# facebookresearch/param

Hardware: AMD Instinct MI355X
Metric: EmbeddingBag lookups/s + achieved HBM GB/s; all-to-all bus-BW at 1/2/4/8 GPU (higher is better)
Workload: dtype f32

## Files before the change

param_amd/csrc/bwd_sorted_alt.inc:

```
#include <rocprim/device/device_radix_sort.hpp>

namespace pm {
namespace {

template <typename K, bool WEIGHTED>
__global__ void __launch_bounds__(kBlock) build_keys_kernel(const KParams p, K* keys, uint32_t* vals,
                                                            uint32_t* bag_of, int rbits, int tshift, int kbits,
                                                            int64_t phase_bags, int64_t slice_begin, int64_t slice_end) {
    extern __shared__ __attribute__((aligned(16))) char smem[];
    int t, tile;
    block_to_tile(p, t, tile);
    if (t >= p.T) return;
    const int64_t bag0 = static_cast<int64_t>(tile) * p.bags_per_block;
    const int64_t left = p.B - bag0;
    const int nb = left < p.bags_per_block ? static_cast<int>(left) : p.bags_per_block;
    const int64_t g0 = static_cast<int64_t>(t) * p.B + bag0;
    int64_t* s_off = reinterpret_cast<int64_t*>(smem);
    for (int i = threadIdx.x; i <= nb; i += kBlock) s_off[i] = bag_start_or_end(p, g0 + i);
    __syncthreads();
    const int64_t base = s_off[0];
    const int64_t end = s_off[nb];
    const K pad = static_cast<K>(1) << kbits;
    for (int64_t j = base + threadIdx.x; j < end; j += kBlock) {
        int lo = 0, hi = nb;
        while (hi - lo > 1) {
            const int mid = (lo + hi) >> 1;
            if (s_off[mid] <= j) lo = mid; else hi = mid;
        }
        const int64_t bag = bag0 + lo;
        const K row = static_cast<K>(load_index(p.indices, j, p.idx64));
        const bool in_slice = bag >= slice_begin && bag < slice_end;
        const K phase = phase_bags > 0 ? static_cast<K>(bag / phase_bags) : static_cast<K>(0);
        keys[j] = in_slice ? ((static_cast<K>(t) << tshift) | (phase << rbits) | row) : pad;
        if (WEIGHTED) {
            vals[j] = static_cast<uint32_t>(j);
            bag_of[j] = static_cast<uint32_t>(bag);
        } else {
            vals[j] = static_cast<uint32_t>(bag);
        }
    }
}

template <typename K>
hipError_t rocprim_temp_bytes(int64_t n, int kbits_sort, size_t& bytes) {
    bytes = 0;
    K* kn = nullptr;
    uint32_t* vn = nullptr;
    return rocprim::radix_sort_pairs(nullptr, bytes, kn, kn, vn, vn, static_cast<size_t>(n), 0u,
                                     static_cast<unsigned>(kbits_sort), hipStream_t(0));
}

std::atomic<int> g_sort_impl{-1}, g_sort_order{-1}, g_max_phases{-1};
void set_alt_tuning(int sort_impl, int order, int max_phases_) {
    g_sort_impl.store(sort_impl);
    g_sort_order.store(order);
    g_max_phases.store(max_phases_);
}
int sort_impl_knob() { return knob(g_sort_impl, [] { return env_is("PARAM_AMD_SORT", "rocprim") ? 1 : env_is("PARAM_AMD_SORT", "legacy") ? 2 : 0; }); }
bool fused_keys_allowed() { return !env_is("PARAM_AMD_SORT_FUSED_KEYS", "0"); }
bool table_major_order() { return knob(g_sort_order, [] { return env_is("PARAM_AMD_SORT_ORDER", "row") ? 0 : 1; }) == 1; }
int max_phases() { return knob(g_max_phases, [] { return env_is("PARAM_AMD_BWD_PHASES", "2") ? 2 : 1; }); }

hipError_t alt_temp_bytes(int64_t n, int, int key_bytes, int kbits_sort, size_t& tb) {
    hipError_t rc = key_bytes == 4 ? rocprim_temp_bytes<uint32_t>(n, kbits_sort > 32 ? 32 : kbits_sort, tb)
                                   : rocprim_temp_bytes<uint64_t>(n, kbits_sort, tb);
    if (rc != hipSuccess) return rc;
    const size_t own = rs_scratch_bytes(static_cast<size_t>(n));
    if (own > tb) tb = own;
    return hipSuccess;
}

void legacy_plan(const KParams& p, int64_t fixed_pooling, int phases, SortPlan& g) {
    const bool fixed = fixed_pooling > 0 && !g.sliced && p.T >= 1 && p.B > 0 &&
                       fixed_pooling * p.B * static_cast<int64_t>(p.T) == p.N;
    g.H = 1;
    if (phases == 2 && max_phases() >= 2 && fixed && table_major_order() && p.B % 2 == 0 && ((p.B / 2) * fixed_pooling) % kSortTile == 0) g.H = 2;
    g.hbits = g.H == 2 ? 1 : 0;
    g.tshift = g.rbits + g.hbits;
    g.kbits = g.tshift + bits_for(p.T);
    g.key_bytes = (g.kbits + 1 <= 32) ? 4 : 8;
    g.phase_bags = g.H == 2 ? p.B / 2 : 0;
    g.seg_len = fixed ? (p.B / g.H) * fixed_pooling : 0;
    g.seg_tiles = (fixed && table_major_order() && g.seg_len % kSortTile == 0) ? static_cast<int32_t>(g.seg_len / kSortTile) : 0;
    g.segmented = fixed && table_major_order() && !g.rocprim && g.seg_len > 0 && g.seg_len % 4096 == 0 && g.seg_len / 4096 <= 4096;
    g.xcd = want_xcd() && g.seg_tiles > 0 && p.T > 1;
    if (g.sliced) g.sort_end_bit = g.kbits + 1;
    else if (g.segmented) g.sort_end_bit = g.rbits;
    else g.sort_end_bit = table_major_order() ? g.kbits : g.rbits;
    g.in_b = g.rocprim || (rs_num_passes(0, g.sort_end_bit) % 2 == 1);
    g.fused_keys = g.segmented && g.H == 1 && !g.weighted && !g.sliced && g.sort_end_bit > 0 && fused_keys_allowed();
}

template <typename K>
hipError_t legacy_sort(const KParams& p, const SortPlan& g, SortWs& ws, hipStream_t stream) {
    K* ka = reinterpret_cast<K*>(ws.keys_a);
    K* kb = reinterpret_cast<K*>(ws.keys_b);
    KParams q = p;
    q.bag_begin = 0;
    q.bag_count = p.B;
    q.tiles_per_table = static_cast<int32_t>((p.B + p.bags_per_block - 1) / p.bags_per_block);
    q.xcd_affine = 0;
    const int grid = q.T * q.tiles_per_table;
    const size_t lds = static_cast<size_t>(q.bags_per_block + 2) * sizeof(int64_t);
    hipError_t zrc = hipMemsetAsync(ws.fix_ctl, 0, 4 * sizeof(uint32_t), stream);
    if (zrc != hipSuccess) return zrc;
    const int64_t s0 = p.bag_begin, s1 = p.bag_begin + p.bag_count;
    if (g.fused_keys) {
        const RsSource src{p.indices, p.idx64, g.tshift, static_cast<uint32_t>(g.seg_len / p.B)};
        return rs_sort_pairs<K>(ka, kb, ws.vals_a, ws.vals_b, static_cast<size_t>(p.N), nullptr, 0, g.sort_end_bit, ws.temp, stream,
                                static_cast<size_t>(g.seg_len), &src);
    }
    if (g.weighted)
        hipLaunchKernelGGL((build_keys_kernel<K, true>), dim3(grid), dim3(kBlock), lds, stream, q, ka, ws.vals_a,
                           ws.bag_of, g.rbits, g.tshift, g.kbits, g.phase_bags, s0, s1);
    else
        hipLaunchKernelGGL((build_keys_kernel<K, false>), dim3(grid), dim3(kBlock), lds, stream, q, ka, ws.vals_a,
                           ws.bag_of, g.rbits, g.tshift, g.kbits, g.phase_bags, s0, s1);
    hipError_t rc = hipGetLastError();
    if (rc != hipSuccess) return rc;
    size_t tb = ws.temp_bytes;
    if (g.rocprim)
        return rocprim::radix_sort_pairs(ws.temp, tb, ka, kb, ws.vals_a, ws.vals_b, static_cast<size_t>(p.N), 0u,
                                         static_cast<unsigned>(g.sort_end_bit), stream);
    return rs_sort_pairs<K>(ka, kb, ws.vals_a, ws.vals_b, static_cast<size_t>(p.N), nullptr, 0, g.sort_end_bit, ws.temp, stream,
                            g.segmented ? static_cast<size_t>(g.seg_len) : 0);
}

std::string legacy_plan_describe(const SortPlan& g) {
    const int passes = g.rocprim ? -1 : rs_num_passes(0, g.sort_end_bit);
    char buf[640];
// ... 12 lines not shown
```

param_amd/csrc/bwd_sorted_apply.h:

```cpp
#pragma once

#include <type_traits>

#include "common.h"
#include "fwd_elem.h"

namespace pm {

constexpr int kSortTile = 1024;

constexpr int kExactRun = 256;
constexpr int kFixGrid = 2048;
constexpr int kMaxTablesLds = 1024;

struct ChunkRec {
    uint32_t lead_len;
    uint32_t trail_len;
};

constexpr uint32_t kJoinedBit = 0x80000000u;

struct SortedParams {
    ChunkRec* recs;
    uint32_t* fix_list;
    uint32_t* fix_ctl;
    float* partials;
    int32_t T;
    const void* keys;
    const uint32_t* vals;
    const uint32_t* bag_of;
    void* const* dst;
    const int32_t* dims;
    const int64_t* out_offsets;
    const float* grad;
    const float* psw;
    int64_t out_stride;
    int32_t gblk_shift;
    int64_t gblk_extra;
    int64_t n;
    int32_t rbits;
    int32_t kbits;
    int32_t max_dim;
    int32_t nt_rows;
    float alpha;
    float* const* mom;
    float lr;
    float eps;
    float wd;
    int32_t wd_mode;
    int32_t sr;
    uint64_t sr_seed;
    int32_t exact_run;
    int32_t tshift;
    int32_t seg_tiles;
    int32_t H;
    int32_t phase;
    int32_t tile;
    int32_t xcd;
    const uint32_t* d_n;
    int32_t unique_wgs_per_cu;
    int32_t join_tiles;
    float* const* state;
};


hipError_t bwd_sorted_launch_f32(const SortedParams& sp, int key_bytes, int max_dim, hipStream_t stream);
hipError_t bwd_sorted_launch_bf16(const SortedParams& sp, int key_bytes, int max_dim, hipStream_t stream);
hipError_t bwd_sorted_launch_f16(const SortedParams& sp, int key_bytes, int max_dim, hipStream_t stream);
struct UniqueArgs {
    const HybTable* hyb_tab;
    const uint32_t* bloom;
    void* emit_keys;
    uint32_t* emit_vals;
    int key_bytes;
    uint32_t* tile_cnt;
    size_t tile_cnt_stride;
    int bloom_wbits;
};
hipError_t bwd_unique_launch_f32(const SortedParams& sp, const KParams& kp, const UniqueArgs& ua, int max_dim, hipStream_t stream);
hipError_t bwd_unique_launch_bf16(const SortedParams& sp, const KParams& kp, const UniqueArgs& ua, int max_dim, hipStream_t stream);
hipError_t bwd_unique_launch_f16(const SortedParams& sp, const KParams& kp, const UniqueArgs& ua, int max_dim, hipStream_t stream);

struct RestArgs {
    const HybTable* hyb_tab;
    int T_h;
    const uint32_t* stage;
    const uint32_t* rest_n;
    const uint32_t* rbits;
    int rbits_stride;
    int parts;
};
int rest_parts(int T_h, int tiles_per_table);
hipError_t bwd_rest_launch_f32(const SortedParams& sp, const KParams& kp, const RestArgs& ra, int max_dim, hipStream_t stream);
hipError_t bwd_rest_launch_bf16(const SortedParams& sp, const KParams& kp, const RestArgs& ra, int max_dim, hipStream_t stream);
hipError_t bwd_rest_launch_f16(const SortedParams& sp, const KParams& kp, const RestArgs& ra, int max_dim, hipStream_t stream);

}
```

param_amd/csrc/embbag_bwd_sorted.hip:

```cpp
#include <atomic>
#include <climits>
#include <cstdint>
#include <cstdio>
#include <cstdlib>
#include <mutex>
#include <string>
#include <unordered_map>
#include <vector>

#include "bwd_sorted_apply.h"

namespace pm {
namespace {

constexpr int kDefaultSortMode = 0;

struct SortWs {
    char* keys_a;
    char* keys_b;
    uint32_t* vals_a;
    uint32_t* vals_b;
    uint32_t* bag_of;
    ChunkRec* recs;
    uint32_t* fix_list;
// ... 20 lines not shown
inline size_t align256(size_t x) { return (x + 255) / 256 * 256; }

inline int bits_for(int64_t n_values) {
    int b = 0;
    while ((static_cast<int64_t>(1) << b) < n_values) ++b;
    return b;
}

std::atomic<int> g_bwd_xcd{-1};
int env_is(const char* name, const char* value) {
    const char* e = getenv(name);
    return (e && std::string(e) == value) ? 1 : 0;
}
template <typename F>
int knob(std::atomic<int>& k, F env_default) {
    int v = k.load();
    if (v < 0) {
        v = env_default();
        k.store(v);
    }
    return v;
}
std::atomic<int> g_sort_mode{-1};
int sort_mode_knob() {
    int v = g_sort_mode.load();
    if (v < 0) {
        const char* e = getenv("PARAM_AMD_SORT_MODE");
        v = (e && e[0] >= '0' && e[0] <= '3') ? e[0] - '0' : kDefaultSortMode;
        g_sort_mode.store(v);
    }
    return v;
}
std::atomic<int> g_hyb_enable{-1};
std::atomic<uint32_t> g_spin_cap{0};
int env_int(const char* name, int dflt) {
    const char* e = getenv(name);
    return (e && e[0] >= '0' && e[0] <= '9') ? atoi(e) : dflt;
}
int hyb_enable_knob() { return knob(g_hyb_enable, [] { return env_int("PARAM_AMD_BWD_HYBRID", 1); }); }
std::atomic<int> g_hyb_rest{-1};
std::atomic<int> g_hyb_min_tiles{-1};
int hyb_rest_knob() { return knob(g_hyb_rest, [] { return env_int("PARAM_AMD_HYB_REST", 1) != 0 ? 1 : 0; }); }
bool want_xcd() { return knob(g_bwd_xcd, [] { return env_is("PARAM_AMD_BWD_XCD", "0") ? 0 : 1; }) == 1; }

struct SortPlan {
    int key_bytes, rbits, hbits, tshift, kbits;
    bool sliced, weighted, rocprim, segmented, in_b, xcd, fused_keys;
    int H;
    int64_t n, seg_len, phase_bags;
    int sort_end_bit;
    int32_t seg_tiles;
    int32_t T;
    bool v2;
    int mode;
    int hyb;
    bool applied;
    bool relabelled;
    bool sequence;
    const void* indices;
    const void* offsets;
    int64_t B, bag_begin, bag_count;
    uint64_t stamp;
};

}
}

#ifdef PM_ALTERNATES
#include "bwd_sorted_alt.inc"
#else
namespace pm {
namespace {
int sort_impl_knob() { return 0; }
void set_alt_tuning(int, int, int) {}
hipError_t alt_temp_bytes(int64_t, int T, int, int, size_t& tb) {
    tb = 0;
    return T > kSegSortMaxTables ? hipErrorInvalidValue : hipSuccess;
}
void legacy_plan(const KParams&, int64_t, int, SortPlan&) {}
template <typename K>
hipError_t legacy_sort(const KParams&, const SortPlan&, SortWs&, hipStream_t) { return hipErrorInvalidValue; }
std::string legacy_plan_describe(const SortPlan&) { return "sort=none"; }
}
}
#endif

namespace pm {
namespace {

template <typename F>
hipError_t with_key_type(int key_bytes, F&& f) {
    return key_bytes == 4 ? f(uint32_t{}) : f(uint64_t{});
}

SortWs ws_layout(const KParams& p, int64_t max_rows, int max_dim, bool weighted, void* base) {
    const int64_t n = p.N;
    const int kbits_sort = bits_for(max_rows) + 1 + bits_for(p.T) + 1;
    const int key_bytes = kbits_sort <= 32 ? 4 : 8;
    SortWs ws{};
    size_t tb = 0;
    if ((ws.rc = alt_temp_bytes(n, p.T, key_bytes, kbits_sort, tb)) != hipSuccess) return ws;
    if (p.T <= kSegSortMaxTables) {
        const size_t seg = seg_sort_scratch_bytes(static_cast<size_t>(n), p.T, !weighted);
        if (seg > tb) tb = seg;
    }
    char* b = reinterpret_cast<char*>(base);
    size_t off = 0;
    auto take = [&](size_t bytes) { char* q = b ? b + off : nullptr; off += align256(bytes); return q; };
    ws.keys_a = take(static_cast<size_t>(n) * key_bytes);
    ws.keys_b = take(static_cast<size_t>(n) * key_bytes);
    ws.vals_a = reinterpret_cast<uint32_t*>(take(static_cast<size_t>(n) * 4));
    ws.vals_b = reinterpret_cast<uint32_t*>(take(static_cast<size_t>(n) * 4));
    ws.bag_of = reinterpret_cast<uint32_t*>(take(weighted ? static_cast<size_t>(n) * 4 : 0));
    const size_t nch = static_cast<size_t>(max_chunks(n, max_dim));
    ws.recs = reinterpret_cast<ChunkRec*>(take(nch * sizeof(ChunkRec)));
    ws.fix_list = reinterpret_cast<uint32_t*>(take(nch * sizeof(uint32_t)));
    ws.fix_ctl = reinterpret_cast<uint32_t*>(take(4 * sizeof(uint32_t)));
    ws.partials = reinterpret_cast<float*>(take(nch * 2 * static_cast<size_t>(max_dim) * sizeof(float)));
    ws.temp = take(tb);
    ws.temp_bytes = tb;
    ws.total = off;
    return ws;
}

SortPlan make_plan(const KParams& p, int64_t max_rows, int64_t fixed_pooling, int phases, bool sequence = false) {
    SortPlan g;
    g.sequence = sequence;
    g.T = p.T;
    g.n = p.N;
    g.rbits = bits_for(max_rows);
    g.sliced = !(p.bag_begin == 0 && p.bag_count == p.B);
    g.weighted = p.psw != nullptr;
    g.rocprim = sort_impl_knob() == 1;
    g.indices = p.indices;
    g.offsets = p.offsets;
    g.B = p.B;
    g.bag_begin = p.bag_begin;
    g.bag_count = p.bag_count;
    g.stamp = 0;
    g.v2 = sort_impl_knob() == 0 && p.T <= kSegSortMaxTables;
    g.mode = sort_mode_knob();
    g.hyb = 0;
    g.applied = false;
    g.relabelled = false;
    g.H = 1;
    g.hbits = 0;
    g.tshift = g.rbits;
    g.kbits = g.tshift + bits_for(p.T);
    g.key_bytes = (g.kbits + 1 <= 32) ? 4 : 8;
    g.phase_bags = 0;
    g.seg_len = 0;
    g.seg_tiles = 0;
    g.segmented = g.v2;
    g.xcd = g.v2 && want_xcd();
    g.sort_end_bit = g.v2 ? g.rbits : g.kbits;
    g.in_b = g.v2 && seg_sort_result_in_b(g.mode, g.rbits);
    g.fused_keys = g.v2 && !g.weighted;
    if (!g.v2) legacy_plan(p, fixed_pooling, phases, g);
    return g;
}

std::mutex g_plan_mutex;
std::unordered_map<const void*, SortPlan> g_plans;
uint64_t g_plan_stamp = 0;

SegSortRequest seg_request(const KParams& p, const SortPlan& g, SortWs& ws) {
    SegSortRequest rq;
    rq.indices = p.indices;
    rq.offsets = p.offsets;
    rq.rows = p.rows;
    rq.idx64 = p.idx64;
    rq.T = p.T;
    rq.B = p.B;
    rq.N = p.N;
    rq.bag_begin = p.bag_begin;
    rq.bag_count = p.bag_count;
    rq.tshift = g.tshift;
    rq.rbits_max = g.rbits;
    rq.weighted = g.weighted;
    rq.sequence = g.sequence;
    rq.zero4 = ws.fix_ctl;
    rq.hyb.allow = g.hyb;
    rq.hyb.slices = hyb_slices(p.N, p.T);
    rq.queue_a = ws.vals_a;
    rq.queue_b = ws.vals_b;
    rq.spin_cap = g_spin_cap.load();
    return rq;
}

template <typename K>
hipError_t sort_impl(const KParams& p, const SortPlan& g, SortWs& ws, hipStream_t stream) {
    if (!g.v2) return legacy_sort<K>(p, g, ws, stream);
    const SegSortRequest rq = seg_request(p, g, ws);
    const hipError_t rc = seg_sort_part_a<K>(rq, ws.temp, stream);
    if (rc != hipSuccess || g.hyb) return rc;
    return seg_sort_part_b<K>(rq, g.mode, reinterpret_cast<K*>(ws.keys_a), reinterpret_cast<K*>(ws.keys_b), ws.vals_a, ws.vals_b, ws.bag_of,
                              ws.temp, stream);
}

template <typename F>
PlanStatus find_plan(const void* workspace, const KParams& p, int64_t max_rows, bool match, SortPlan& out, F&& follow_up) {
    std::lock_guard<std::mutex> lock(g_plan_mutex);
    auto it = g_plans.find(workspace);
    if (it == g_plans.end()) return PlanStatus::none;
    SortPlan& g = it->second;
// ... 108 lines not shown
}

PlanStatus sorted_pairs_info(const KParams& p, int64_t max_rows, int max_dim, const void* workspace, SortedPairsInfo& out) {
    SortPlan g;
    if (find_plan(workspace, p, max_rows, false, g, [](SortPlan&) { return PlanStatus::ok; }) != PlanStatus::ok) return PlanStatus::none;
    out.deferred = g.hyb && !g.applied;
    if (out.deferred) return PlanStatus::ok;
    const SortWs ws = ws_layout(p, max_rows, max_dim, g.weighted, const_cast<void*>(workspace));
    if (ws.rc != hipSuccess) return PlanStatus::none;
    out.keys = g.in_b ? ws.keys_b : ws.keys_a;
    out.vals = g.in_b ? ws.vals_b : ws.vals_a;
    out.d_count = g.v2 ? seg_sort_view(ws.temp, static_cast<size_t>(p.N), p.T).n_total : nullptr;
    out.key_bytes = g.key_bytes;
    out.tshift = g.tshift;
    return PlanStatus::ok;
}

hipError_t bwd_sorted_apply(const KParams& p, int64_t max_rows, int dst_dtype, int max_dim, const void* workspace, hipStream_t stream,
                            ApplyUpdate update) {
    SortPlan g;
    if (find_plan(workspace, p, max_rows, false, g, [](SortPlan& r) { r.applied = true; return PlanStatus::ok; }) != PlanStatus::ok)
        return hipErrorInvalidValue;
    SortWs ws = ws_layout(p, max_rows, max_dim, g.weighted, const_cast<void*>(workspace));
    if (ws.rc != hipSuccess) return ws.rc;
    if (p.T > kMaxTablesLds) return hipErrorInvalidValue;
    const SegScratchView sv = seg_sort_view(ws.temp, static_cast<size_t>(p.N), p.T);
    const pm_rowwise_adagrad* opt = update.opt;
    SortedParams sp;
    sp.recs = ws.recs;
    sp.fix_list = ws.fix_list;
    sp.fix_ctl = ws.fix_ctl;
    sp.partials = ws.partials;
    sp.T = p.T;
    sp.keys = g.in_b ? ws.keys_b : ws.keys_a;
    sp.vals = g.in_b ? ws.vals_b : ws.vals_a;
    sp.bag_of = ws.bag_of;
    sp.dst = const_cast<void* const*>(p.tables);
    sp.dims = p.dims;
    sp.out_offsets = g.sequence ? nullptr : p.out_offsets;
    sp.grad = p.io;
    sp.psw = p.psw;
    sp.out_stride = p.out_stride;
    sp.gblk_shift = p.gblk_shift;
    sp.gblk_extra = p.gblk_extra;
    sp.n = p.N;
    sp.rbits = g.rbits;
    sp.kbits = g.kbits;
    sp.tshift = g.tshift;
    sp.max_dim = max_dim;
    sp.nt_rows = p.nt_loads;
    sp.alpha = p.alpha;
    sp.mom = update.elementwise ? nullptr : update.state;
    sp.state = update.elementwise ? update.state : nullptr;
    sp.lr = opt ? opt->lr : 0.0f;
    sp.eps = opt ? opt->eps : 0.0f;
    sp.wd = opt ? opt->weight_decay : 0.0f;
    sp.wd_mode = opt ? opt->weight_decay_mode : PM_WD_NONE;
    sp.sr = (opt && opt->stochastic_rounding && dst_dtype != PM_F32) ? 1 : 0;
    sp.sr_seed = opt ? opt->seed : 0;
    sp.exact_run = kExactRun;
    sp.seg_tiles = (!g.v2 && (g.xcd || g.H > 1)) ? g.seg_tiles : 0;
    sp.H = g.H;
    sp.phase = 0;
    sp.xcd = g.xcd ? (g.v2 ? 2 : 1) : 0;
    sp.d_n = g.v2 ? sv.n_total : nullptr;
    sp.tile = g.v2 ? apply_tile(p.N) : kSortTile;
    sp.unique_wgs_per_cu = 0;
    if (sp.n == 0) return hipSuccess;
    const ApplyLaunchers& launch = kApplyLaunchers[dst_dtype == PM_F32 ? 0 : dst_dtype == PM_BF16 ? 1 : 2];
    if (g.sequence && (g.hyb || sp.psw || sp.gblk_extra != 0)) return hipErrorInvalidValue;
    if (!g.hyb) return launch.sorted(sp, g.key_bytes, max_dim, stream);
    UniqueArgs ua;
    ua.hyb_tab = sv.hyb_tab;
    ua.bloom = sv.bloom;
    ua.emit_keys = ws.keys_b;
    ua.emit_vals = ws.vals_b;
    ua.key_bytes = g.key_bytes;
    ua.tile_cnt = sv.tile_cnt;
    ua.tile_cnt_stride = sv.tile_cnt_stride;
    ua.bloom_wbits = bloom_wbits(hyb_slices(p.N, p.T));
    KParams q = p;
    q.bags_per_block = kUniqueBags;
    q.tiles_per_table = static_cast<int32_t>((q.bag_count + kUniqueBags - 1) / kUniqueBags);
    q.idx_cap = 4096;
    if (q.tiles_per_table < 1 || q.tiles_per_table > kCompactMaxTiles) return hipErrorInvalidValue;
    hipError_t rc = launch.unique(sp, q, ua, max_dim, stream);
    if (rc != hipSuccess) return rc;
    const int rest_mode = hyb_rest_knob();
    const HybTiles tiles{q.bags_per_block, q.tiles_per_table};
    rc = with_key_type(g.key_bytes, [&](auto k) {
        using K = decltype(k);
        return seg_sort_stage_leftovers<K>(seg_request(p, g, ws), reinterpret_cast<const K*>(ws.keys_b), ws.vals_b,
                                           reinterpret_cast<K*>(ws.keys_a), ws.vals_a, tiles, rest_mode != 0 ? 1 : 0, ws.temp, stream);
    });
    if (rc != hipSuccess) return rc;
    if (rest_mode != 0) {
        RestArgs ra;
        ra.hyb_tab = ua.hyb_tab;
        ra.T_h = p.T < kHybMaxTables ? p.T : kHybMaxTables;
        ra.stage = sv.rest_stage;
        ra.rest_n = sv.rest_n;
        ra.rbits = &sv.desc->rbits;
        ra.rbits_stride = static_cast<int>(sizeof(SegDesc) / sizeof(uint32_t));
        ra.parts = rest_parts(ra.T_h, q.tiles_per_table);
        if ((rc = launch.rest(sp, q, ra, max_dim, stream)) != hipSuccess) return rc;
    }
// ... 44 lines not shown
```

param_amd/csrc/embbag_bwd_sorted_kernels.inc:

```

template <typename DST, int G>
__device__ __forceinline__ void adagrad_finish(char* wptr, float (&wrow)[DST::kVec], const float (&acc)[DST::kVec],
                                               bool any_col, float* mom_row, float mom_prev, int D, const SortedParams& p,
                                               int lig, int nt_rows, uint64_t rowkey, int c) {
    float ss = 0.0f;
    if (p.wd_mode == PM_WD_L2) {
#pragma unroll
        for (int k = 0; k < DST::kVec; ++k) {
            const float reg = any_col ? p.wd * wrow[k] : 0.0f;
            const float gx = acc[k] + reg;
            ss = ss + gx * gx;
        }
    } else {
#pragma unroll
        for (int k = 0; k < DST::kVec; ++k) ss = ss + acc[k] * acc[k];
    }
#pragma unroll
    for (int off = G / 2; off >= 1; off >>= 1) ss = ss + __shfl_xor(ss, off, G);
    const float m = mom_prev + ss / static_cast<float>(D);
    if (lig == 0) hidden_store4(mom_row, m);
    const float mult = p.lr / (sqrtf(m) + p.eps);
    if (any_col) {
        if (p.wd_mode != PM_WD_NONE) {
            const float shrink = p.wd_mode == PM_WD_L2 ? mult * p.wd : p.lr * p.wd;
// ... 47 lines not shown
__device__ __forceinline__ void state_load_raw(const void* p, u32x4 (&raw)[VEC / 4], int nt_rows) {
#pragma unroll
    for (int k = 0; k < VEC / 4; ++k) raw[k] = raw16_load(reinterpret_cast<const char*>(p) + 16 * k, nt_rows);
}
template <int VEC>
__device__ __forceinline__ void state_widen(const u32x4 (&raw)[VEC / 4], float (&st)[VEC]) {
#pragma unroll
    for (int k = 0; k < VEC / 4; ++k) {
        st[4 * k] = __uint_as_float(raw[k].x); st[4 * k + 1] = __uint_as_float(raw[k].y);
        st[4 * k + 2] = __uint_as_float(raw[k].z); st[4 * k + 3] = __uint_as_float(raw[k].w);
    }
}

template <typename DST, int G, int OPT>
__device__ __forceinline__ void finish_row(char* wptr, float (&wrow)[DST::kVec], float (&acc)[DST::kVec], const float (&srow)[OPT == 2 ? DST::kVec : 1],
                                           bool cols, float* state, float m_prev, int D, const SortedParams& p, int lig, int nt_rows,
                                           uint64_t rowkey, int c) {
    if constexpr (OPT == 2) {
        if (cols) adagrad_elem_finish<DST>(wptr, wrow, acc, srow, state, p, nt_rows, rowkey, c);
    } else
    if (OPT == 1) adagrad_finish<DST, G>(wptr, wrow, acc, cols, state, m_prev, D, p, lig, nt_rows, rowkey, c);
    else if (cols) DST::store(wptr, acc, nt_rows);
}
template <int VEC, typename P>
__device__ __forceinline__ void load_grad(P g, float (&gv)[VEC]) {
#pragma unroll
    for (int k = 0; k < VEC; k += 4) {
        const f32x4 x = g[k / 4];
        gv[k] = x.x; gv[k + 1] = x.y; gv[k + 2] = x.z; gv[k + 3] = x.w;
    }
}
template <int VEC>
__device__ __forceinline__ void add_scaled(float (&acc)[VEC], float sc, const float (&gv)[VEC]) {
#pragma unroll
    for (int k = 0; k < VEC; ++k) {
        const float prod = sc * gv[k];
        acc[k] = acc[k] + prod;
    }
}
template <typename DST, int OPT>
__device__ __forceinline__ void open_row(const u32x4 raw, const u32x4 (&sraw)[OPT == 2 ? DST::kVec / 4 : 1], float (&acc)[DST::kVec],
                                         float (&wrow)[DST::kVec], float (&srow)[OPT == 2 ? DST::kVec : 1]) {
    float wv[DST::kVec];
    DST::widen(raw, wv);
#pragma unroll
    for (int k = 0; k < DST::kVec; ++k) {
        if (OPT != 0) wrow[k] = wv[k];
        else acc[k] = wv[k];
    }
    if constexpr (OPT == 2) state_widen<DST::kVec>(sraw, srow);
}
template <int OPT, int VEC>
__device__ __forceinline__ int column_pass_end(int lig, int width) { return OPT != 0 ? lig * VEC + 1 : width; }

template <int G>
__device__ __forceinline__ int group_first(bool pred) {
    const uint64_t m = __ballot(pred);
    if (G == 64) return m ? __builtin_ctzll(m) : G;
    const int sh = (threadIdx.x & 63) / G * G;
    const uint64_t gm = (m >> sh) & ((1ull << (G & 63)) - 1ull);
    return gm ? __builtin_ctzll(gm) : G;
}
template <int G, typename K>
__device__ __forceinline__ int count_same_lds_fwd(const K* s_key, int from, int to, K key) {
    const int lig = threadIdx.x % G;
    for (int j0 = 0; j0 < to - from; j0 += G) {
        const int j = j0 + lig;
        const bool differs = (from + j >= to) || s_key[from + j + 1] != key;
        const int f = group_first<G>(differs);
        if (f < G) return (j0 + f < to - from) ? j0 + f : to - from;
    }
    return to - from;
}
template <int G, typename K>
__device__ __forceinline__ int count_same_lds_bwd(const K* s_key, int from, int to, K key) {
    const int lig = threadIdx.x % G;
    for (int j0 = 0; j0 < to - from; j0 += G) {
        const int j = j0 + lig;
        const bool differs = (to - 1 - j < from) || s_key[to - j] != key;
        const int f = group_first<G>(differs);
        if (f < G) return (j0 + f < to - from) ? j0 + f : to - from;
    }
    return to - from;
}

#ifndef PM_RUN_DEEP
#define PM_RUN_DEEP 2
#endif
template <typename DST, typename K, int G, bool WEIGHTED, int OPT, int TILE>
__global__ void __launch_bounds__(kBlock) bwd_sorted_main_kernel(const SortedParams p) {
    const uint32_t fix_gen = p.fix_ctl[2];
    if (blockIdx.x == 0 && threadIdx.x == 0) p.fix_ctl[3] = fix_gen;
    PM_STAMP(blockIdx.x, 0);
#ifndef PM_KBATCH_F32
#define PM_KBATCH_F32 4
#endif
#ifndef PM_KBATCH_16
#define PM_KBATCH_16 2
#endif
    constexpr bool kLean = OPT == 2 && DST::kES == 2;
    constexpr int kBatch = DST::kES == 2 ? (kLean ? 1 : PM_KBATCH_16) : PM_KBATCH_F32;
    constexpr int kDeepMul = kLean ? 4 : PM_RUN_DEEP;
    constexpr int VEC = DST::kVec;
    constexpr int NG = kBlock / G;
    constexpr int C = TILE / NG;
    constexpr int kOver = kExactRun;
    __shared__ K s_keyw[TILE + 2 + 2 * kOver];
    __shared__ uint32_t s_val[TILE + kOver];
    K* const s_key = s_keyw + kOver;
    extern __shared__ __attribute__((aligned(16))) char s_tab[];
    char** s_dst = reinterpret_cast<char**>(s_tab);
    int64_t* s_ooff = reinterpret_cast<int64_t*>(s_tab + static_cast<size_t>(p.T) * 8);
    float** s_mom = reinterpret_cast<float**>(s_tab + static_cast<size_t>(p.T) * 16);
    int32_t* s_dim = reinterpret_cast<int32_t*>(s_tab + static_cast<size_t>(p.T) * (OPT != 0 ? 24 : 16));

    const K* keys = reinterpret_cast<const K*>(p.keys);
    const int nt_rows = p.nt_rows;
    const K pad_bit = static_cast<K>(1) << p.kbits;
    const K row_mask = (static_cast<K>(1) << p.rbits) - 1;
    const int64_t n_sorted = p.d_n ? static_cast<int64_t>(*p.d_n) : p.n;
    int64_t tile_id = blockIdx.x;
    if (p.xcd == 2) {
        const int64_t per = ((n_sorted + TILE - 1) / TILE + kXcds - 1) / kXcds;
        const int64_t slot = blockIdx.x / kXcds;
        if (slot >= per) return;
        tile_id = (blockIdx.x % kXcds) * per + slot;
    } else if (p.seg_tiles > 0) {
        int64_t t, i;
        if (p.xcd) {
            const int xcd = blockIdx.x % kXcds;
            const int64_t slot = blockIdx.x / kXcds;
            t = xcd + kXcds * (slot / p.seg_tiles);
            i = slot % p.seg_tiles;
        } else {
            t = blockIdx.x / p.seg_tiles;
            i = blockIdx.x % p.seg_tiles;
        }
        if (t >= p.T) return;
        tile_id = (t * p.H + p.phase) * p.seg_tiles + i;
    }
    const int64_t base = tile_id * TILE;
    if (base >= n_sorted) return;
    const int n_tile = (n_sorted - base) < TILE ? static_cast<int>(n_sorted - base) : TILE;
    const int nb = base < kOver ? static_cast<int>(base) : kOver;
    const int64_t after = n_sorted - (base + n_tile);
    const int nf = after < kOver ? static_cast<int>(after) : kOver;
    for (int i = static_cast<int>(threadIdx.x) - nb; i < n_tile + nf; i += kBlock) {
        s_key[i + 1] = keys[base + i];
        if (i >= 0) s_val[i] = p.vals[base + i];
    }
    if (threadIdx.x == 0) {
        s_key[-nb] = base - nb > 0 ? keys[base - nb - 1] : pad_bit;
        s_key[n_tile + nf + 1] = (base + n_tile + nf < n_sorted) ? keys[base + n_tile + nf] : pad_bit;
    }
    for (int t = threadIdx.x; t < p.T; t += kBlock) {
        s_dst[t] = reinterpret_cast<char*>(p.dst[t]);
        s_ooff[t] = p.out_offsets ? p.out_offsets[t] : 0;
        s_dim[t] = p.dims[t];
        if (OPT == 1) s_mom[t] = p.mom[t];
        if (OPT == 2) s_mom[t] = p.state[t];
    }
    __syncthreads();
    PM_STAMP(blockIdx.x, 1);
    constexpr bool kJoin = !(WEIGHTED && OPT != 0);
    __shared__ float s_join[kJoin ? kBlock * VEC : 1];
    const bool tile_joined = kJoin && p.join_tiles && n_tile == TILE && s_key[1] == s_key[TILE] && s_key[0] == s_key[1] &&
                             s_key[TILE + 1] == s_key[1] && !(s_key[1] & pad_bit);

    const int gid = threadIdx.x / G;
    const int lig = threadIdx.x % G;
    const int l0 = gid * C;
    if (l0 >= n_tile) return;
    const int l1 = (l0 + C < n_tile) ? l0 + C : n_tile;
    const int64_t chunk = (base / TILE) * NG + gid;
    ChunkRec* rec = p.recs + chunk;
    float* lead_slot = p.partials + (chunk * 2) * p.max_dim;
    float* trail_slot = lead_slot + p.max_dim;

    const K first_key = s_key[l0 + 1];
    const K last_key = s_key[l1];
    const bool lead_open = first_key == s_key[l0] && !(first_key & pad_bit);
    const bool trail_open = last_key == s_key[l1 + 1] && !(last_key & pad_bit);

    int lead_skip = 0, own_after = 0;
    bool lead_partial = lead_open, trail_partial = trail_open;
    if (p.exact_run > 0 && (lead_open || trail_open)) {
        bool whole_chunk_in_lead_run = false;
        if (lead_open) {
            const int in_chunk = count_same_lds_fwd<G, K>(s_key, l0, l1, first_key);
            const bool goes_on = in_chunk == l1 - l0 && trail_open;
            whole_chunk_in_lead_run = goes_on;
            const int right = goes_on ? count_same_lds_fwd<G, K>(s_key, l1, n_tile + nf, first_key) : 0;
            const int before = count_same_lds_bwd<G, K>(s_key, -nb, l0, first_key);
            const bool leaves_tile = (before == l0 + nb && s_key[-nb] == first_key) ||
                                     (goes_on && l1 + right == n_tile + nf && s_key[n_tile + nf + 1] == first_key);
            if (!leaves_tile && before + in_chunk + right <= p.exact_run) {
                lead_skip = in_chunk;
                lead_partial = false;
                if (goes_on) trail_partial = false;
            }
        }
        if (trail_open && !whole_chunk_in_lead_run) {
            const int tail = count_same_lds_bwd<G, K>(s_key, l0, l1, last_key);
            const int right = count_same_lds_fwd<G, K>(s_key, l1, n_tile + nf, last_key);
            const bool leaves_tile = l1 + right == n_tile + nf && s_key[n_tile + nf + 1] == last_key;
            if (!leaves_tile && tail + right <= p.exact_run) {
                own_after = right;
                trail_partial = false;
            }
        }
    }

    const int l1e = l1 + own_after;
    PM_STAMP(blockIdx.x, 2);

    const int c_end = column_pass_end<OPT, VEC>(lig, p.max_dim);
    for (int c = lig * VEC; c < c_end; c += G * VEC) {
        int mode = 0;
        bool any_col = false, done = false;
        int seg_start = l0;
        uint32_t lead_len = 0, trail_len = 0;
        float acc[VEC];
        float wrow[VEC];
        float cur_mom = 0.0f;
        constexpr int SV = OPT == 2 ? VEC : 1;
        float srow[SV];
        K cur_key = 0;
#pragma unroll
        for (int k = 0; k < VEC; ++k) { acc[k] = 0.0f; wrow[k] = 0.0f; }
#pragma unroll
        for (int k = 0; k < SV; ++k) srow[k] = 0.0f;
        const char* const dummy_fast = reinterpret_cast<const char*>(p.partials) + static_cast<size_t>(lig) * VEC * sizeof(float);
        auto close_run = [&](K key, float (&a)[VEC], float (&w)[VEC], bool cols, float m_prev) {
            const int t = static_cast<int>(key >> p.tshift);
            const int64_t row = static_cast<int64_t>(key & row_mask);
            const int D = s_dim[t];
            char* wptr = s_dst[t] + (row * D + c) * DST::kES;
            if constexpr (OPT == 2) {
                if (cols) adagrad_elem_finish<DST>(wptr, w, a, srow, s_mom[t] + row * D + c, p, nt_rows, static_cast<uint64_t>(key), c);
            } else
            if (OPT == 1) adagrad_finish<DST, G>(wptr, w, a, cols, s_mom[t] + row, m_prev, D, p, lig, nt_rows, static_cast<uint64_t>(key), c);
            else if (cols) DST::store(wptr, a, nt_rows);
        };
        for (int pos = l0 + lead_skip; pos < l1e && !done; pos += kBatch) {
            K kk[kBatch + 1];
            uint32_t vv[kBatch];
            bool valid[kBatch], head[kBatch];
            if (!WEIGHTED && mode != 0 && pos + kBatch <= l1e) {
                bool same = true;
#pragma unroll
                for (int u = 0; u < kBatch; ++u) same = same && s_key[pos + u + 1] == cur_key;
                if (same) {
                    const int t = static_cast<int>(cur_key >> p.tshift);
                    const float* gt = any_col ? p.grad + s_ooff[t] + c : reinterpret_cast<const float*>(dummy_fast);
                    const int64_t stride = any_col ? p.out_stride : 0;
                    const int64_t bextra = any_col ? p.gblk_extra : 0;
                    constexpr int kDeep = kDeepMul * kBatch;
                    bool deep = kDeepMul > 1 && pos + kDeep <= l1e;
#pragma unroll
                    for (int u = kBatch; u < kDeep; ++u) deep = deep && s_key[pos + (u < kDeep ? u : 0) + 1] == cur_key;
                    if (deep) {
                        float gf[kDeep][VEC];
#pragma unroll
                        for (int u = 0; u < kDeep; ++u) {
                            const float* g = gt + grad_bag_offset(static_cast<int64_t>(s_val[pos + u]), stride, p.gblk_shift, bextra);
#pragma unroll
                            for (int k = 0; k < VEC; k += 4) {
                                const f32x4 x = *reinterpret_cast<const f32x4*>(g + k);
                                gf[u][k] = x.x; gf[u][k + 1] = x.y; gf[u][k + 2] = x.z; gf[u][k + 3] = x.w;
                            }
                        }
                        if (any_col) {
#pragma unroll
                            for (int u = 0; u < kDeep; ++u)
#pragma unroll
                                for (int k = 0; k < VEC; ++k) {
                                    const float prod = p.alpha * gf[u][k];
                                    acc[k] = acc[k] + prod;
                                }
                        }
                        pos += kDeep - kBatch;
                        continue;
                    }
                    float gf[kBatch][VEC];
#pragma unroll
                    for (int u = 0; u < kBatch; ++u) {
                        const float* g = gt + grad_bag_offset(static_cast<int64_t>(s_val[pos + u]), stride, p.gblk_shift, bextra);
#pragma unroll
                        for (int k = 0; k < VEC; k += 4) {
                            const f32x4 x = *reinterpret_cast<const f32x4*>(g + k);
                            gf[u][k] = x.x; gf[u][k + 1] = x.y; gf[u][k + 2] = x.z; gf[u][k + 3] = x.w;
                        }
                    }
                    if (any_col) {
#pragma unroll
                        for (int u = 0; u < kBatch; ++u)
#pragma unroll
                            for (int k = 0; k < VEC; ++k) {
                                const float prod = p.alpha * gf[u][k];
                                acc[k] = acc[k] + prod;
                            }
                    }
                    continue;
                }
            }
            kk[0] = s_key[pos];
#pragma unroll
            for (int u = 0; u < kBatch; ++u) {
                const bool in = (pos + u) < l1e;
                kk[u + 1] = in ? s_key[pos + u + 1] : pad_bit;
                valid[u] = in && !(kk[u + 1] & pad_bit);
                vv[u] = valid[u] ? s_val[pos + u] : 0u;
                head[u] = valid[u] && kk[u + 1] != kk[u];
            }
            float gv[kBatch][VEC];
            u32x4 wraw[kBatch];
            float sc[kBatch];
            float mv[kBatch];
            u32x4 sraw[kBatch][OPT == 2 ? VEC / 4 : 1];
            bool col_ok[kBatch];
            const char* const dummy = reinterpret_cast<const char*>(p.partials) + static_cast<size_t>(lig) * VEC * sizeof(float);
#pragma unroll
            for (int u = 0; u < kBatch; ++u) {
                mv[u] = 0.0f;
                const K key = kk[u + 1];
                const int t = valid[u] ? static_cast<int>(key >> p.tshift) : 0;
                const int64_t row = static_cast<int64_t>(key & row_mask);
                const int D = s_dim[t];
                col_ok[u] = valid[u] && c < D;
                const bool need_row = col_ok[u] && head[u] && !(trail_partial && key == last_key);
                if (OPT == 1 && valid[u] && head[u] && !(trail_partial && key == last_key)) mv[u] = *as_global<float>(s_mom[t] + row);
                uint32_t bag = vv[u];
                sc[u] = p.alpha;
                if (WEIGHTED) {
                    if (col_ok[u]) {
                        sc[u] = p.alpha * p.psw[vv[u]];
                        bag = p.bag_of[vv[u]];
                    }
                }
                const float* g = col_ok[u] ? p.grad + s_ooff[t] + grad_bag_offset(static_cast<int64_t>(bag), p.out_stride, p.gblk_shift, p.gblk_extra) + c
                                           : reinterpret_cast<const float*>(dummy);
                load_grad<VEC>(reinterpret_cast<const f32x4*>(g), gv[u]);
                wraw[u] = DST::load_raw(need_row ? s_dst[t] + (row * D + c) * DST::kES : dummy, nt_rows);
                if constexpr (OPT == 2)
                    state_load_raw<VEC>(need_row ? reinterpret_cast<const char*>(s_mom[t] + row * D + c) : dummy, sraw[u], nt_rows);
            }
#pragma unroll
            for (int u = 0; u < kBatch; ++u) {
                if (done) break;
                if (!valid[u]) {
                    done = true;
                    break;
                }
                const int q = pos + u;
                if (head[u] || (q == l0 && lead_partial)) {
                    if (mode == 2) {
                        close_run(cur_key, acc, wrow, any_col, cur_mom);
                    }
                    if (mode == 1) {
                        lead_len = static_cast<uint32_t>(q - l0);
                        if (any_col) {
                            hidden_store_vec<VEC>(lead_slot + c, acc);
                        }
                    }
                    seg_start = q;
                    any_col = col_ok[u];
                    cur_key = kk[u + 1];
                    cur_mom = mv[u];
                    if (!head[u]) {
                        mode = 1;
                    } else if (trail_partial && kk[u + 1] == last_key) {
                        mode = 3;
                    } else {
                        mode = 2;
                    }
#pragma unroll
                    for (int k = 0; k < VEC; ++k) acc[k] = 0.0f;
                    if (mode == 2 && any_col) open_row<DST, OPT>(wraw[u], sraw[u], acc, wrow, srow);
                }
                if (mode != 0 && any_col) add_scaled<VEC>(acc, sc[u], gv[u]);
            }
#pragma unroll
            for (int u = 0; u < kBatch; ++u) {
#pragma unroll
                for (int k = 0; k < VEC; ++k) asm volatile("" : : "v"(gv[u][k]));
                asm volatile("" : : "v"(wraw[u]));
                asm volatile("" : : "v"(mv[u]), "v"(sc[u]));
                if constexpr (OPT == 2) {
#pragma unroll
                    for (int k = 0; k < VEC / 4; ++k) asm volatile("" : : "v"(sraw[u][k]));
                }
            }
        }
        if (mode == 2) {
            close_run(cur_key, acc, wrow, any_col, cur_mom);
        }
        if (mode == 1) {
            int real = l1 - l0;
            while (real > 0 && (s_key[l0 + real] & pad_bit)) --real;
            lead_len = static_cast<uint32_t>(real);
            if (any_col && !tile_joined) {
                hidden_store_vec<VEC>(lead_slot + c, acc);
            }
        }
        if (tile_joined) {
            float* const sj = s_join + threadIdx.x * VEC;
#pragma unroll
            for (int k = 0; k < VEC; ++k) sj[k] = acc[k];
            __syncthreads();
            if (gid == 0) {
                float sum[VEC];
#pragma unroll
                for (int k = 0; k < VEC; ++k) sum[k] = acc[k];
#pragma unroll 1
                for (int g = 1; g < NG; ++g) {
#pragma unroll
                    for (int k = 0; k < VEC; ++k) sum[k] = sum[k] + s_join[(g * G + lig) * VEC + k];
                }
                if (any_col) hidden_store_vec<VEC>(lead_slot + c, sum);
            }
            if (c + G * VEC < c_end) __syncthreads();
        }
        if (mode == 3) {
            trail_len = static_cast<uint32_t>(l1 - seg_start);
            if (any_col) {
                hidden_store_vec<VEC>(trail_slot + c, acc);
            }
        }
        if (c == 0 && lig == 0) {
            rec->lead_len = lead_len | ((tile_joined && gid == 0) ? kJoinedBit : 0u);
            rec->trail_len = trail_len;
            if (trail_len > 0) p.fix_list[atomicAdd(p.fix_ctl + (fix_gen & 1u), 1u)] = static_cast<uint32_t>(chunk);
        }
    }
    PM_STAMP_DRAINED(blockIdx.x, 3);
}

template <typename DST, typename K, int G, bool WEIGHTED, int OPT, int TILE>
__device__ __forceinline__ void fixup_one_run(const SortedParams& p, int64_t h, uint32_t trail, int64_t walk_end, uint32_t* my_bag, float* my_sc) {
    constexpr int VEC = DST::kVec;
    constexpr int NG = kBlock / G;
    constexpr int C = TILE / NG;
    constexpr int kFixBatch = 128 / VEC;
    const int lig = threadIdx.x % G;

    const int nt_rows = p.nt_rows;
    const K* keys = reinterpret_cast<const K*>(p.keys);
    const K row_mask = (static_cast<K>(1) << p.rbits) - 1;
    const int64_t c1 = (h + 1) * C;
    const int64_t start = c1 - trail;
    const K key = keys[start];
    const int t = static_cast<int>(key >> p.tshift);
    const int64_t row = static_cast<int64_t>(key & row_mask);
    const int D = p.dims[t];

    int64_t len = trail, last = h;
    int64_t jt0 = 0;
    int64_t njt = 0;
    bool tiles_done = !p.join_tiles;
    for (int64_t i0 = h + 1; i0 < walk_end;) {
        if (!tiles_done && i0 % NG == 0) {
            const int64_t i = i0 + static_cast<int64_t>(lig) * NG;
            const uint32_t ll = i < walk_end ? p.recs[i].lead_len : 0u;
            const int f = group_first<G>(!(ll & kJoinedBit));
            const int full = f < G ? f : G;
            if (njt == 0) jt0 = i0;
            njt += full;
            len += static_cast<int64_t>(full) * TILE;
            i0 += static_cast<int64_t>(full) * NG;
            if (full > 0) last = i0 - 1;
            tiles_done = f < G;
            continue;
        }
        int n = G;
        if (!tiles_done) {
            const int64_t to_border = (i0 / NG + 1) * NG - i0;
            if (to_border < n) n = static_cast<int>(to_border);
        }
        const int64_t i = i0 + lig;
        const uint32_t ll = lig >= n ? static_cast<uint32_t>(C) : (i < walk_end ? p.recs[i].lead_len : 0u);
        const int f = group_first<G>(ll < static_cast<uint32_t>(C));
        const int full = f < G ? f : n;
        len += static_cast<int64_t>(full) * C;
        last = i0 + full - 1;
        if (f < G) {
            const uint32_t tail = __shfl(ll, f, G);
            if (tail > 0) {
// ... 544 lines not shown
```

Measured before the change: 22.14 billion.

## Specialize sorted-backward apply for tiles whose keys all belong to one table

Adds a table_major flag to the sort plan and apply params, and makes the apply kernel check whether a tile's keys all come from one table. If so, it skips the per-block LDS fill of table metadata and its barrier, resolves the table once as a wave-uniform value, and uses 32-bit offset arithmetic for gradient and state addressing. Chunk-record and partial-slot pointers are recomputed when needed instead of being held live. The intent is to cut LDS lookups, 64-bit address math and register pressure in the hot loop, at the cost of two instantiations of the column-pass body (larger code) and a 32-bit range assumption guarded by a stride check.

Result: no change. 22.15 billion, median of 3 (+0.0%).

```diff
diff --git a/param_amd/csrc/bwd_sorted_alt.inc b/param_amd/csrc/bwd_sorted_alt.inc
--- a/param_amd/csrc/bwd_sorted_alt.inc
+++ b/param_amd/csrc/bwd_sorted_alt.inc
@@ -76,6 +76,7 @@
     g.H = 1;
     if (phases == 2 && max_phases() >= 2 && fixed && table_major_order() && p.B % 2 == 0 && ((p.B / 2) * fixed_pooling) % kSortTile == 0) g.H = 2;
     g.hbits = g.H == 2 ? 1 : 0;
+    g.table_major = table_major_order();
     g.tshift = g.rbits + g.hbits;
     g.kbits = g.tshift + bits_for(p.T);
     g.key_bytes = (g.kbits + 1 <= 32) ? 4 : 8;
diff --git a/param_amd/csrc/bwd_sorted_apply.h b/param_amd/csrc/bwd_sorted_apply.h
--- a/param_amd/csrc/bwd_sorted_apply.h
+++ b/param_amd/csrc/bwd_sorted_apply.h
@@ -61,6 +61,7 @@
     int32_t unique_wgs_per_cu;
     int32_t join_tiles;
     float* const* state;
+    int32_t table_major;
 };
 
 
diff --git a/param_amd/csrc/embbag_bwd_sorted.hip b/param_amd/csrc/embbag_bwd_sorted.hip
--- a/param_amd/csrc/embbag_bwd_sorted.hip
+++ b/param_amd/csrc/embbag_bwd_sorted.hip
@@ -96,6 +96,7 @@
     int32_t seg_tiles;
     int32_t T;
     bool v2;
+    bool table_major;
     int mode;
     int hyb;
     bool applied;
@@ -195,6 +196,7 @@
     g.phase_bags = 0;
     g.seg_len = 0;
     g.seg_tiles = 0;
+    g.table_major = true;
     g.segmented = g.v2;
     g.xcd = g.v2 && want_xcd();
     g.sort_end_bit = g.v2 ? g.rbits : g.kbits;
@@ -409,6 +411,7 @@
     sp.alpha = p.alpha;
     sp.mom = update.elementwise ? nullptr : update.state;
     sp.state = update.elementwise ? update.state : nullptr;
+    sp.table_major = g.table_major ? 1 : 0;
     sp.lr = opt ? opt->lr : 0.0f;
     sp.eps = opt ? opt->eps : 0.0f;
     sp.wd = opt ? opt->weight_decay : 0.0f;
diff --git a/param_amd/csrc/embbag_bwd_sorted_kernels.inc b/param_amd/csrc/embbag_bwd_sorted_kernels.inc
--- a/param_amd/csrc/embbag_bwd_sorted_kernels.inc
+++ b/param_amd/csrc/embbag_bwd_sorted_kernels.inc
@@ -123,6 +123,27 @@
 }
 template <int OPT, int VEC>
 __device__ __forceinline__ int column_pass_end(int lig, int width) { return OPT != 0 ? lig * VEC + 1 : width; }
+
+struct TableRef {
+    int D;
+    char* dst;
+    int64_t ooff;
+    float* state;
+};
+template <int OPT>
+__device__ __forceinline__ TableRef resolve_table(const SortedParams& p, int t) {
+    TableRef r;
+    r.D = p.dims[t];
+    r.dst = reinterpret_cast<char*>(p.dst[t]);
+    r.ooff = p.out_offsets ? p.out_offsets[t] : 0;
+    r.state = OPT == 1 ? p.mom[t] : OPT == 2 ? p.state[t] : nullptr;
+    return r;
+}
+template <typename P>
+__device__ __forceinline__ P* at_u32(P* base, uint32_t index, uint32_t factor_bytes) {
+    using C = std::conditional_t<std::is_const_v<P>, const char, char>;
+    return reinterpret_cast<P*>(reinterpret_cast<C*>(base) + static_cast<uint64_t>(index) * factor_bytes);
+}
 
 template <int G>
 __device__ __forceinline__ int group_first(bool pred) {
@@ -224,14 +245,22 @@
         s_key[-nb] = base - nb > 0 ? keys[base - nb - 1] : pad_bit;
         s_key[n_tile + nf + 1] = (base + n_tile + nf < n_sorted) ? keys[base + n_tile + nf] : pad_bit;
     }
-    for (int t = threadIdx.x; t < p.T; t += kBlock) {
-        s_dst[t] = reinterpret_cast<char*>(p.dst[t]);
-        s_ooff[t] = p.out_offsets ? p.out_offsets[t] : 0;
-        s_dim[t] = p.dims[t];
-        if (OPT == 1) s_mom[t] = p.mom[t];
-        if (OPT == 2) s_mom[t] = p.state[t];
-    }
     __syncthreads();
+    const K tile_k0 = s_key[1], tile_k1 = s_key[n_tile];
+    const bool tile_one_table = __builtin_amdgcn_readfirstlane(
+        static_cast<int>(p.table_major != 0 && !(tile_k1 & pad_bit) && (tile_k0 >> p.tshift) == (tile_k1 >> p.tshift) &&
+                         p.gblk_extra == 0 && p.out_stride >= 0 && p.out_stride < (static_cast<int64_t>(1) << 30))) != 0;
+    const int tile_t = __builtin_amdgcn_readfirstlane(static_cast<int>(tile_k0 >> p.tshift));
+    if (!tile_one_table) {
+        for (int t = threadIdx.x; t < p.T; t += kBlock) {
+            const TableRef r = resolve_table<OPT>(p, t);
+            s_dst[t] = r.dst;
+            s_ooff[t] = r.ooff;
+            s_dim[t] = r.D;
+            if (OPT != 0) s_mom[t] = r.state;
+        }
+        __syncthreads();
+    }
     PM_STAMP(blockIdx.x, 1);
     constexpr bool kJoin = !(WEIGHTED && OPT != 0);
     __shared__ float s_join[kJoin ? kBlock * VEC : 1];
@@ -244,9 +273,13 @@
     if (l0 >= n_tile) return;
     const int l1 = (l0 + C < n_tile) ? l0 + C : n_tile;
     const int64_t chunk = (base / TILE) * NG + gid;
-    ChunkRec* rec = p.recs + chunk;
-    float* lead_slot = p.partials + (chunk * 2) * p.max_dim;
-    float* trail_slot = lead_slot + p.max_dim;
+    auto chunk_here = [&]() -> int64_t {
+        int g = gid;
+        asm volatile("" : "+v"(g));
+        return (base / TILE) * NG + g;
+    };
+    auto lead_slot_at = [&](int c) -> float* { return p.partials + (chunk_here() * 2) * p.max_dim + c; };
+    auto trail_slot_at = [&](int c) -> float* { return p.partials + (chunk_here() * 2 + 1) * p.max_dim + c; };
 
     const K first_key = s_key[l0 + 1];
     const K last_key = s_key[l1];
@@ -285,6 +318,12 @@
     const int l1e = l1 + own_after;
     PM_STAMP(blockIdx.x, 2);
 
+    auto column_passes = [&](auto uni) {
+    constexpr bool UNI = decltype(uni)::value;
+    TableRef tile_tab{0, nullptr, 0, nullptr};
+    if constexpr (UNI) tile_tab = resolve_table<OPT>(p, tile_t);
+    const uint32_t state_bytes = static_cast<uint32_t>(tile_tab.D) * static_cast<uint32_t>(sizeof(float));
+    const uint32_t stride_bytes = static_cast<uint32_t>(p.out_stride) * static_cast<uint32_t>(sizeof(float));
     const int c_end = column_pass_end<OPT, VEC>(lig, p.max_dim);
     for (int c = lig * VEC; c < c_end; c += G * VEC) {
         int mode = 0;
@@ -302,15 +341,28 @@
 #pragma unroll
         for (int k = 0; k < SV; ++k) srow[k] = 0.0f;
         const char* const dummy_fast = reinterpret_cast<const char*>(p.partials) + static_cast<size_t>(lig) * VEC * sizeof(float);
+        auto row_ptr = [&](const TableRef& tr, int64_t row) -> char* { return tr.dst + (row * tr.D + c) * DST::kES; };
+        auto state_ptr = [&](const TableRef& tr, int64_t row) -> float* {
+            if constexpr (OPT == 1) return tr.state + row;
+            else if constexpr (UNI) return at_u32(tr.state + c, static_cast<uint32_t>(row), state_bytes);
+            else return tr.state + row * tr.D + c;
+        };
+        auto table_of = [&](K key, bool valid) -> TableRef {
+            if constexpr (UNI) return tile_tab;
+            else {
+                const int t = valid ? static_cast<int>(key >> p.tshift) : 0;
+                return TableRef{s_dim[t], s_dst[t], s_ooff[t], OPT != 0 ? s_mom[t] : nullptr};
+            }
+        };
         auto close_run = [&](K key, float (&a)[VEC], float (&w)[VEC], bool cols, float m_prev) {
-            const int t = static_cast<int>(key >> p.tshift);
+            const TableRef tr = table_of(key, true);
             const int64_t row = static_cast<int64_t>(key & row_mask);
-            const int D = s_dim[t];
-            char* wptr = s_dst[t] + (row * D + c) * DST::kES;
+            const int D = tr.D;
+            char* wptr = row_ptr(tr, row);
             if constexpr (OPT == 2) {
-                if (cols) adagrad_elem_finish<DST>(wptr, w, a, srow, s_mom[t] + row * D + c, p, nt_rows, static_cast<uint64_t>(key), c);
+                if (cols) adagrad_elem_finish<DST>(wptr, w, a, srow, state_ptr(tr, row), p, nt_rows, static_cast<uint64_t>(key), c);
             } else
-            if (OPT == 1) adagrad_finish<DST, G>(wptr, w, a, cols, s_mom[t] + row, m_prev, D, p, lig, nt_rows, static_cast<uint64_t>(key), c);
+            if (OPT == 1) adagrad_finish<DST, G>(wptr, w, a, cols, state_ptr(tr, row), m_prev, D, p, lig, nt_rows, static_cast<uint64_t>(key), c);
             else if (cols) DST::store(wptr, a, nt_rows);
         };
         for (int pos = l0 + lead_skip; pos < l1e && !done; pos += kBatch) {
@@ -322,10 +374,14 @@
 #pragma unroll
                 for (int u = 0; u < kBatch; ++u) same = same && s_key[pos + u + 1] == cur_key;
                 if (same) {
-                    const int t = static_cast<int>(cur_key >> p.tshift);
-                    const float* gt = any_col ? p.grad + s_ooff[t] + c : reinterpret_cast<const float*>(dummy_fast);
+                    const float* gt = any_col ? p.grad + table_of(cur_key, true).ooff + c : reinterpret_cast<const float*>(dummy_fast);
                     const int64_t stride = any_col ? p.out_stride : 0;
                     const int64_t bextra = any_col ? p.gblk_extra : 0;
+                    const uint32_t stride_b = any_col ? stride_bytes : 0u;
+                    auto run_grad = [&](uint32_t bag) -> const float* {
+                        if constexpr (UNI) return at_u32(gt, bag, stride_b);
+                        else return gt + grad_bag_offset(static_cast<int64_t>(bag), stride, p.gblk_shift, bextra);
+                    };
                     constexpr int kDeep = kDeepMul * kBatch;
                     bool deep = kDeepMul > 1 && pos + kDeep <= l1e;
 #pragma unroll
@@ -334,7 +390,7 @@
                         float gf[kDeep][VEC];
 #pragma unroll
                         for (int u = 0; u < kDeep; ++u) {
-                            const float* g = gt + grad_bag_offset(static_cast<int64_t>(s_val[pos + u]), stride, p.gblk_shift, bextra);
+                            const float* g = run_grad(s_val[pos + u]);
 #pragma unroll
                             for (int k = 0; k < VEC; k += 4) {
                                 const f32x4 x = *reinterpret_cast<const f32x4*>(g + k);
@@ -356,7 +412,7 @@
                     float gf[kBatch][VEC];
 #pragma unroll
                     for (int u = 0; u < kBatch; ++u) {
-                        const float* g = gt + grad_bag_offset(static_cast<int64_t>(s_val[pos + u]), stride, p.gblk_shift, bextra);
+                        const float* g = run_grad(s_val[pos + u]);
 #pragma unroll
                         for (int k = 0; k < VEC; k += 4) {
                             const f32x4 x = *reinterpret_cast<const f32x4*>(g + k);
@@ -395,12 +451,11 @@
             for (int u = 0; u < kBatch; ++u) {
                 mv[u] = 0.0f;
                 const K key = kk[u + 1];
-                const int t = valid[u] ? static_cast<int>(key >> p.tshift) : 0;
+                const TableRef tr = table_of(key, valid[u]);
                 const int64_t row = static_cast<int64_t>(key & row_mask);
-                const int D = s_dim[t];
-                col_ok[u] = valid[u] && c < D;
+                col_ok[u] = valid[u] && c < tr.D;
                 const bool need_row = col_ok[u] && head[u] && !(trail_partial && key == last_key);
-                if (OPT == 1 && valid[u] && head[u] && !(trail_partial && key == last_key)) mv[u] = *as_global<float>(s_mom[t] + row);
+                if (OPT == 1 && valid[u] && head[u] && !(trail_partial && key == last_key)) mv[u] = *as_global<float>(state_ptr(tr, row));
                 uint32_t bag = vv[u];
                 sc[u] = p.alpha;
                 if (WEIGHTED) {
@@ -409,12 +464,14 @@
                         bag = p.bag_of[vv[u]];
                     }
                 }
-                const float* g = col_ok[u] ? p.grad + s_ooff[t] + grad_bag_offset(static_cast<int64_t>(bag), p.out_stride, p.gblk_shift, p.gblk_extra) + c
-                                           : reinterpret_cast<const float*>(dummy);
+                const float* g;
+                if constexpr (UNI) g = col_ok[u] ? at_u32(p.grad + tr.ooff + c, bag, stride_bytes) : reinterpret_cast<const float*>(dummy);
+                else g = col_ok[u] ? p.grad + tr.ooff + grad_bag_offset(static_cast<int64_t>(bag), p.out_stride, p.gblk_shift, p.gblk_extra) + c
+                                   : reinterpret_cast<const float*>(dummy);
                 load_grad<VEC>(reinterpret_cast<const f32x4*>(g), gv[u]);
-                wraw[u] = DST::load_raw(need_row ? s_dst[t] + (row * D + c) * DST::kES : dummy, nt_rows);
+                wraw[u] = DST::load_raw(need_row ? row_ptr(tr, row) : dummy, nt_rows);
                 if constexpr (OPT == 2)
-                    state_load_raw<VEC>(need_row ? reinterpret_cast<const char*>(s_mom[t] + row * D + c) : dummy, sraw[u], nt_rows);
+                    state_load_raw<VEC>(need_row ? reinterpret_cast<const char*>(state_ptr(tr, row)) : dummy, sraw[u], nt_rows);
             }
 #pragma unroll
             for (int u = 0; u < kBatch; ++u) {
@@ -431,7 +488,7 @@
                     if (mode == 1) {
                         lead_len = static_cast<uint32_t>(q - l0);
                         if (any_col) {
-                            hidden_store_vec<VEC>(lead_slot + c, acc);
+                            hidden_store_vec<VEC>(lead_slot_at(c), acc);
                         }
                     }
                     seg_start = q;
@@ -471,7 +528,7 @@
             while (real > 0 && (s_key[l0 + real] & pad_bit)) --real;
             lead_len = static_cast<uint32_t>(real);
             if (any_col && !tile_joined) {
-                hidden_store_vec<VEC>(lead_slot + c, acc);
+                hidden_store_vec<VEC>(lead_slot_at(c), acc);
             }
         }
         if (tile_joined) {
@@ -488,22 +545,26 @@
 #pragma unroll
                     for (int k = 0; k < VEC; ++k) sum[k] = sum[k] + s_join[(g * G + lig) * VEC + k];
                 }
-                if (any_col) hidden_store_vec<VEC>(lead_slot + c, sum);
+                if (any_col) hidden_store_vec<VEC>(lead_slot_at(c), sum);
             }
             if (c + G * VEC < c_end) __syncthreads();
         }
         if (mode == 3) {
             trail_len = static_cast<uint32_t>(l1 - seg_start);
             if (any_col) {
-                hidden_store_vec<VEC>(trail_slot + c, acc);
+                hidden_store_vec<VEC>(trail_slot_at(c), acc);
             }
         }
         if (c == 0 && lig == 0) {
+            ChunkRec* rec = p.recs + chunk_here();
             rec->lead_len = lead_len | ((tile_joined && gid == 0) ? kJoinedBit : 0u);
             rec->trail_len = trail_len;
             if (trail_len > 0) p.fix_list[atomicAdd(p.fix_ctl + (fix_gen & 1u), 1u)] = static_cast<uint32_t>(chunk);
         }
     }
+    };
+    if (!tile_one_table) column_passes(std::false_type{});
+    else column_passes(std::true_type{});
     PM_STAMP_DRAINED(blockIdx.x, 3);
 }
 
```
